# calavera/patrol

Hardware: AMD Instinct MI355X
Metric: bucket-state merges/sec + achieved HBM GB/s at 1/2/4/8 MI355X (higher is better)
Workload: dtype f64; 1 GPU; C2 merge: 100000000 replica messages -> 10000000-bucket table (2^25 slots), Zipf(1.1); keys_per_gpu=10000000, slots_per_gpu=33554432, parallelism=shard1, name_bytes=2-8 (b<id>), world_size=1, full=False, exchange=False, batches_in_hbm=28

## Files before the change

### patrol_amd/csrc/phip_engine.hip

```cpp
#include <sys/random.h>

#include <chrono>
#include <cstdlib>
#include <cstring>
#include <hip/hip_runtime.h>
#include <rocprim/rocprim.hpp>

#include <algorithm>
#include <cstdarg>
#include <cstdio>
#include <cstring>
#include <mutex>
#include <string>
#include <vector>

#include "patrolhip.h"
#include "phip_kernels.hpp"
#include "phip_host.hpp"

using namespace phip;

namespace {

#ifndef PHIP_SORT_BITS
// ... 29 lines not shown
struct DevBuf {
  void* p = nullptr;
  size_t cap = 0;
};

struct Timing {
  const char* name;
  hipEvent_t a, b;
};

}

struct phip_handle {
  int device = 0;
  int ncu = 256;
  u32 ndef = 0;
  bool iso_always = false;
  u32 iso_left = 0;
  bool coll_iso = false;
  bool classify_first = false;
  u32 opt_left = 0;
  struct LastStats {
    uint64_t hot_entries = 0, hot_hits = 0, misses = 0;
    uint64_t ordered = 0;
    uint64_t log_count = 0, log_over = 0;
  } stats;
  hipStream_t stream = nullptr;
  hipStream_t own_stream = nullptr;
  hipStream_t stream2 = nullptr;
  hipStream_t stream3 = nullptr;
  hipStream_t stream4 = nullptr;
  hipEvent_t ev_t4a = nullptr, ev_t4b = nullptr;
  hipEvent_t ev_fork = nullptr, ev_join = nullptr;
  hipEvent_t ev_fork3 = nullptr, ev_join3 = nullptr;
  hipEvent_t ev_gather = nullptr, ev_gather3 = nullptr;
  hipEvent_t ev_pack = nullptr;
  std::mutex mu;
  std::string err;
  u32 L = 0;
  u32 L_open = 0;
  u64 cap = 0;
  u64 max_load = 0;
  u32 load_pct = 90;
  bool grow = true;
  bool small = true;
  u64 grows = 0;
  u64 layout_gen = 1;
  u64 long_need = 0;
  Rec* recs = nullptr;
  u32* aux = nullptr;
  u8* arena = nullptr;
  u64 arena_cap = 0;
  u64 arena_open = 0;
  u64* arena_cursor = nullptr;
  u32* ctr = nullptr;
  u32* ctr_host = nullptr;
  u32* ctr_map = nullptr;
  u32 fpar = 0;
  u64 nfast = 0;
  u64 n_buckets = 0;
  u64 tag_mask = ~0ull;
  u64 seed = 0;
  DevBuf buf[B_COUNT_];
  bool timing = false;
  bool timing_accumulate = false;
  std::vector<Timing> timings;
// ... 336 lines not shown
    cur = nxt;
    nxt = (nxt == retry) ? spare : retry;
  }
  *n_claimed = total;
  if (h->long_need) {
    if ((rc = read_ctr(h)) || (rc = check_flags(h))) return rc;
  }
  return PHIP_OK;
}

int clear_new(phip_handle* h, u32 n_claimed) {
  if (!n_claimed) return PHIP_OK;
  u32* cslot = (u32*)h->buf[B_CSLOT].p;
  Launch l(h, "k_clear_new");
  k_clear_new<<<grid_for(n_claimed), kBlock, 0, h->stream>>>(cslot, n_claimed, table(h));
  HIPCHK(h, hipGetLastError());
  return PHIP_OK;
}

int after_error(phip_handle* h, int rc) {
  if (rc == PHIP_OK) return rc;
  if (h->stream2) (void)hipStreamSynchronize(h->stream2);
  if (h->stream3) (void)hipStreamSynchronize(h->stream3);
  if (h->stream4) (void)hipStreamSynchronize(h->stream4);
  if (rc == PHIP_ERR_HIP) return rc;
  std::string keep = h->err;
  k_clear_new_all<<<grid_for(h->cap), kBlock, 0, h->stream>>>(table(h), h->cap);
  if (hipGetLastError() == hipSuccess) (void)hipStreamSynchronize(h->stream);
  h->err = keep;
  return rc;
}

template <class Src>
int build_hot(phip_handle* h, Src src, u32 n, hipStream_t st, const HotHdr** hdr_out,
              const HotEntry** dir_out) {
  *hdr_out = nullptr;
  *dir_out = nullptr;
  if (n < kHotMinBatch) return PHIP_OK;
  constexpr size_t kCnt = size_t(1) << kHotCntBits;
  const size_t zero_bytes = 2 * kCnt * sizeof(u32) + kHotHist * sizeof(u32) + sizeof(HotHdr);
  u8* base;
  int rc;
  if ((rc = ensure(h, B_HOT, zero_bytes + kHotMax * sizeof(HotEntry), &base))) return rc;
  u32* ckeys = (u32*)base;
  u32* ccnt = ckeys + kCnt;
  u32* hist = ccnt + kCnt;
  HotHdr* hdr = (HotHdr*)(hist + kHotHist);
  HotEntry* dir = (HotEntry*)(hdr + 1);
  HIPCHK(h, hipMemsetAsync(base, 0, zero_bytes, st));
  const u32 stride = std::max<u32>(64, (n + kHotSampleMax - 1) / kHotSampleMax);
  const u32 nsample = (n + stride - 1) / stride;
  {
    Launch l(h, "k_hot_sample", st);
    k_hot_sample<Src><<<grid_for(nsample, kHotSamplePerBlock), 256, 0, st>>>(
        src, n, stride, nsample, table(h), ckeys, ccnt);
  }
  {
    Launch l(h, "k_hot_select", st);
    k_hot_hist<<<grid_for(kCnt), kBlock, 0, st>>>(ccnt, hist);
    k_hot_select<<<1, 256, 0, st>>>(hist, hdr, kHotMax);
    k_hot_build<<<grid_for(kCnt), kBlock, 0, st>>>(ckeys, ccnt, hdr, table(h), dir);
  }
  HIPCHK(h, hipGetLastError());
  *hdr_out = hdr;
  *dir_out = dir;
  return PHIP_OK;
}

inline unsigned fast_grid_on(u32 ncu, u32 n) {
  const u64 tiles = ((u64)n + kFastBlock - 1) / kFastBlock;
  return (unsigned)std::max<u64>(1, std::min<u64>(tiles, (u64)ncu * kFastPerCU));
}
inline unsigned fast_grid(phip_handle* h, u32 n) { return fast_grid_on((u32)h->ncu, n); }

int join_hot(phip_handle* h, const HotHdr* hot);

int sharded(phip_handle* h, BufId base_id, u32 units, u32 per_unit, Sharded* out,
            bool zero = true) {
  int rc;
  out->cap = shard_cap(units, per_unit);
  if ((rc = ensure(h, base_id, (size_t)kShards * out->cap, &out->base)) ||
      (rc = ensure(h, B_MSCNT, 2 * kShards, &out->cnt)))
    return rc;
  if (zero) HIPCHK(h, hipMemsetAsync(out->cnt, 0, kShards * sizeof(u32), h->stream));
  return PHIP_OK;
}

int pack_sharded(phip_handle* h, const Sharded& sh, u32 total_slot, u32* out, u32* total) {
  k_shard_scan<<<1, kShards, 0, h->stream>>>(sh.cnt, h->ctr, total_slot, nullptr, 0, nullptr,
                                             nullptr);
  HIPCHK(h, hipGetLastError());
  int rc;
  if ((rc = read_ctr(h))) return rc;
  *total = h->ctr_host[total_slot];
  if (*total) {
    Launch l(h, "k_shard_compact");
    dim3 grid(grid_for(h->ctr_host[kCtrShardMax]), kShards);
    k_shard_compact<<<grid, 256, 0, h->stream>>>(sh.base, sh.cap, sh.cnt, out);
    HIPCHK(h, hipGetLastError());
  }
  return PHIP_OK;
}

template <class Src>
int fork_hot(phip_handle* h, Src src, u32 n, const HotHdr** hot, const HotEntry** hot_dir);

struct FastFront {
  const HotHdr* hot = nullptr;
  const HotEntry* dir = nullptr;
  u32 par = 0;
  bool iso = false;
  u32* c = nullptr;
  u8* mark = nullptr;
  bool opt = false;
  UndoLog log{};
};

inline bool opt_allowed(const phip_handle* h) {
  return !h->classify_first && h->opt_left == 0 && !h->iso_always && h->iso_left == 0;
}

inline size_t undo_counts(const phip_handle* h) { return (size_t)h->ncu * kFastPerCU * (kFastBlock / 64); }

struct UndoLayout {
  u32 grid, waves, cap;
  u64 halves;
};
inline UndoLayout undo_layout(u32 n, u32 ncu) {
  UndoLayout l;
  l.grid = fast_grid_on(ncu, n);
  l.waves = l.grid * (kFastBlock / 64);
  l.cap = undo_wave_cap(n, l.grid);
  l.halves = (u64)l.waves * l.cap * 2;
  return l;
}

inline u32* fctr(phip_handle* h, u32 par) { return h->ctr + kCtrWords * (1 + par); }

inline u32* fast_counts(phip_handle* h, u32 par) {
  return (u32*)h->buf[B_FSCNT].p + par * 2 * kShards;
}

int dirty_set(phip_handle* h, DirtySet* d, u32** dlist) {
  int rc;
  u64* b;
  if ((rc = ensure(h, B_DTAB, DirtySet::kWords, &b)) || (rc = ensure(h, B_DLIST, kDirtyCap, dlist)))
    return rc;
  *d = DirtySet::at(b);
  return PHIP_OK;
// ... 18 lines not shown
  int rc;
  u32* c;
  out->cap = shard_cap((n + 63) / 64, 64);
  if ((rc = ensure(h, B_MSHARD, (size_t)kShards * out->cap, &out->base)) ||
      (rc = ensure(h, B_FSCNT, 4 * kShards, &c)))
    return rc;
  out->cnt = fast_counts(h, par);
  return PHIP_OK;
}

template <class In, class HotSrc>
int fast_front(phip_handle* h, In in, HotSrc hsrc, u32 n, u8* status, FastFront* ff,
               bool reset = true, int iso = -1, bool opt = false) {
  int rc;
  *ff = FastFront{};
  ff->iso = iso >= 0 ? iso != 0 : (h->iso_always || h->iso_left > 0);
  u32 *c, *dlist = nullptr;
  DirtySet dset;
  if ((rc = ensure(h, B_FSCNT, 4 * kShards, &c))) return rc;
  ff->par = h->fpar ^= 1u;
  ff->c = fctr(h, ff->par);
  ++h->nfast;
  if (reset) {
    k_batch_reset<<<1, kShards, 0, h->stream>>>(ff->c, fast_counts(h, ff->par));
    HIPCHK(h, hipGetLastError());
  }
  if constexpr (In::kSoa) {
    if (opt && iso < 0 && opt_allowed(h)) {
      u32* lc;
      const size_t nw = undo_counts(h);
      if ((rc = ensure(h, B_ULCNT, nw, &lc))) return rc;
      ff->opt = true;
      ff->log.cnt = lc;
      if (n >= kHotMinBatch) HIPCHK(h, hipEventRecord(h->ev_fork, h->stream));
      if (kOptStatus) ff->mark = status;
      else if (status) HIPCHK(h, hipMemsetAsync(status, PHIP_ST_MERGED, n, h->stream));
      if (n >= kHotMinBatch && (rc = fork_hot(h, hsrc, n, &ff->hot, &ff->dir))) return rc;
      return PHIP_OK;
    }
  }
  if ((rc = dirty_set(h, &dset, &dlist))) return rc;
  if (ff->iso) {
    ff->mark = status;
    if (!status) {
      if ((rc = ensure(h, B_DMARK, n, &ff->mark))) return rc;
      HIPCHK(h, hipMemsetAsync(ff->mark, 0, n, h->stream));
    }
  }
  const bool with_hot = n >= kHotMinBatch;
  const bool hot_first = n < (1u << 23);
  if (with_hot) HIPCHK(h, hipEventRecord(h->ev_fork, h->stream));
  if (with_hot && hot_first && (rc = fork_hot(h, hsrc, n, &ff->hot, &ff->dir))) return rc;
  {
    bool done = false;
    if constexpr (In::kSoa) {
      if ((((uintptr_t)in.ma | (uintptr_t)in.mt) & 15) == 0) {
        Launch l(h, "k_classify");
        NamesOffs chk{};
        if constexpr (In::kOffs) chk = in.src;
        k_classify_soa2<<<grid_for((n + 1) / 2), kBlock, 0, h->stream>>>(in.ma, in.mt, in.me, n,
                                                                          ff->c, status, chk,
                                                                          dlist);
        done = true;
      }
    }
    if (!done) {
      if (status) HIPCHK(h, hipMemsetAsync(status, PHIP_ST_MERGED, n, h->stream));
      Launch l(h, "k_classify");
      k_classify<In><<<grid_for(n), kBlock, 0, h->stream>>>(in, n, ff->c, dlist);
    }
  }
  HIPCHK(h, hipGetLastError());
  if (with_hot && !hot_first && (rc = fork_hot(h, hsrc, n, &ff->hot, &ff->dir))) return rc;
  return PHIP_OK;
}

template <class In>
int fast_back(phip_handle* h, In in, u32 n, FastFront& ff, bool queued) {
  u32* miss;
  int rc;
  Sharded msh;
  DirtySet dset{};
  SubBatch sb{};
  u32* dlist = nullptr;
  if ((rc = ensure(h, B_MISS, n, &miss)) || (rc = fast_shards(h, n, ff.par, &msh))) return rc;
  if (ff.iso) {
    if ((rc = dirty_set(h, &dset, &dlist)) || (rc = sub_batch(h, &sb))) return rc;
    Launch l(h, "k_dirty_build");
    k_dirty_build<In><<<1, 1024, 0, h->stream>>>(in, n, ff.c, dlist, dset, table(h));
    HIPCHK(h, hipGetLastError());
  }
  if ((rc = join_hot(h, ff.hot))) return rc;
  if (ff.opt) {
    if constexpr (In::kSoa) {
      const UndoLayout ul = undo_layout(n, (u32)h->ncu);
      ff.log.cap = ul.cap;
      if ((rc = ensure(h, B_ULOG, (size_t)ul.halves, &ff.log.base))) return rc;
      Launch l(h, "k_receive_fast");
      k_receive_fast<In, true><<<ul.grid, kFastBlock, 0, h->stream>>>(
          in, 0, n, table(h), msh, ff.c, ff.hot, ff.dir, nullptr, ff.mark, ff.log);
    }
  } else {
    Launch l(h, "k_receive_fast");
    k_receive_fast<In><<<fast_grid(h, n), kFastBlock, 0, h->stream>>>(
        in, 0, n, table(h), msh, ff.c, ff.hot, ff.dir, ff.iso ? dset.key : nullptr, ff.mark,
        UndoLog{});
  }
  HIPCHK(h, hipGetLastError());
  if (ff.iso) {
    {
      Launch l(h, "k_dirty_pass");
      const unsigned g = (unsigned)std::max<u64>(
          1, std::min<u64>(((u64)n + 1023) / 1024, (u64)h->ncu * 2));
      k_dirty_pass<In><<<g, 1024, 0, h->stream>>>(in, n, ff.c, ff.mark, dset.key, table(h), msh);
      HIPCHK(h, hipGetLastError());
    }
    k_batch_end<In><<<1, kShards, 0, h->stream>>>(
        in, ff.c, dset.key, table(h),
        SubOut{sb.off, sb.len, sb.a, sb.t, sb.e, sb.map, kSubBatchCap}, msh.cnt, h->ctr_map,
        kCtrWords, queued ? fast_counts(h, ff.par ^ 1u) : nullptr, fctr(h, ff.par ^ 1u));
  } else {
    k_shard_scan<<<1, kShards, 0, h->stream>>>(msh.cnt, ff.c, kCtrMiss, h->ctr_map, kCtrWords,
                                               queued ? fast_counts(h, ff.par ^ 1u) : nullptr,
                                               fctr(h, ff.par ^ 1u));
  }
  HIPCHK(h, hipGetLastError());
  HIPCHK(h, hipEventRecord(h->ev_ctr, h->stream));
  if (!queued) HIPCHK(h, hipEventSynchronize(h->ev_ctr));
  return PHIP_OK;
}

constexpr u32 kIsoKeep = 256;
constexpr u32 kOptBackoff = 256;

bool opt_failed(phip_handle* h, u32 n) {
  h->stats.log_count = h->ctr_host[kCtrLogCount];
  h->stats.log_over = h->ctr_host[kCtrLogOver];
  if (h->stats.log_over) h->opt_left = kOptBackoff;
  return h->ctr_host[kCtrDirty] < n || h->ctr_host[kCtrStop] < n || h->stats.log_over != 0;
}

// ... 20 lines not shown
    HIPCHK(h, hipGetLastError());
  }
  const u32 nd = h->ctr_host[kCtrNDirty];
  const bool iso = iso_ran && nd != 0 && nd <= kDirtyCap;
  *first_dirty = iso ? n : std::min<u32>(h->ctr_host[kCtrDirty], n);
  if (h->ctr_host[kCtrDirty] < n) h->iso_left = kIsoKeep;
  else if (h->iso_left) --h->iso_left;
  h->coll_iso = iso_ran;
  h->ndef = iso ? h->ctr_host[kCtrNDefer] : 0;
  h->stats.ordered = 0;
  h->stats.hot_entries = h->ctr_host[kCtrHotEntries];
  h->stats.hot_hits = h->ctr_host[kCtrHotHits];
  h->stats.misses = *nmiss;
  return PHIP_OK;
}

template <class In, class HotSrc>
int fast_apply(phip_handle* h, In in, HotSrc hsrc, u32 n, u8* status, u32* first_dirty,
               u32* nmiss, int iso = -1, bool opt = false) {
  int rc;
  FastFront ff;
  if ((rc = fast_front(h, in, hsrc, n, status, &ff, true, iso, opt)) ||
      (rc = fast_back(h, in, n, ff, false)))
    return rc;
  if (ff.opt && opt_failed(h, n)) {
    if ((rc = undo_pass(h, n, ff.log)) || (rc = fast_front(h, in, hsrc, n, status, &ff, true, iso)) ||
        (rc = fast_back(h, in, n, ff, false)))
      return rc;
  }
  return fast_collect(h, n, ff.par, first_dirty, nmiss, ff.iso, ff.opt);
}

template <class Src>
int fork_hot(phip_handle* h, Src src, u32 n, const HotHdr** hot, const HotEntry** hot_dir);

template <class Src>
int dedupe_names(phip_handle* h, Src src, const u32* list, u32 n, u32** out, u32* nout) {
  int rc;
  u32 setbits = 1;
  while ((1ull << setbits) < 2ull * n) ++setbits;
  u64* set;
  Sharded dsh;
  if ((rc = ensure(h, B_DSET, size_t(1) << setbits, &set)) ||
      (rc = ensure(h, B_DEDUP, n, out)) ||
      (rc = sharded(h, B_MSHARD, grid_for(n), kBlock, &dsh)))
    return rc;
  HIPCHK(h, hipMemsetAsync(set, 0, (size_t(1) << setbits) * sizeof(u64), h->stream));
  {
    Launch l(h, "k_dedupe");
    k_dedupe<Src><<<grid_for(n), kBlock, 0, h->stream>>>(src, n, list, table(h), set, setbits, dsh);
    HIPCHK(h, hipGetLastError());
  }
  return pack_sharded(h, dsh, kCtrAux, *out, nout);
}

template <class Src>
int finish_many_misses(phip_handle* h, Src src, const uint64_t* a, const uint64_t* t,
                       const int64_t* e, u32 nmiss, u32 prefix, i64 now, u8* status, u32* nmiss2) {
  u32* miss = (u32*)h->buf[B_MISS].p;
  int rc;
  u32 *dedup, nd = 0;
  if ((rc = dedupe_names(h, src, miss, nmiss, &dedup, &nd))) return rc;
  u32 n_claimed = 0;
  if ((rc = insert_names(h, src, dedup, nd, nullptr, now, &n_claimed, nullptr, true))) return rc;
  if (status) {
    Launch l(h, "k_first_seen");
    k_first_seen<Src><<<grid_for(nmiss), kBlock, 0, h->stream>>>(src, nmiss, miss, table(h));
    HIPCHK(h, hipGetLastError());
  }
// ... 14 lines not shown
int finish_misses(phip_handle* h, Src src, const uint64_t* a, const uint64_t* t, const int64_t* e,
                  u32 nmiss, u32 prefix, i64 now, u8* status) {
  if (nmiss == 0) return PHIP_OK;
  int rc;
  if (nmiss >= kManyMisses &&
      (rc = finish_many_misses(h, src, a, t, e, nmiss, prefix, now, status, &nmiss)))
    return rc;
  if (nmiss == 0) return PHIP_OK;
  u32* miss = (u32*)h->buf[B_MISS].p;
  u32 n_claimed = 0;
  if ((rc = insert_names(h, src, miss, nmiss, nullptr, now, &n_claimed))) return rc;
  HIPCHK(h, hipMemsetAsync(h->ctr + kCtrMiss, 0, sizeof(u32), h->stream));
  u32* miss2;
  if ((rc = ensure(h, B_MISS2, nmiss, &miss2))) return rc;
  {
    Launch l(h, "k_receive_list");
    k_receive_list<Src><<<grid_for(nmiss), kBlock, 0, h->stream>>>(
        src, a, t, e, nmiss, miss, table(h), status, miss2, h->ctr);
  }
  HIPCHK(h, hipGetLastError());
  {
    Launch l(h, "k_mark_created");
    k_mark_created<Src><<<grid_for(nmiss), kBlock, 0, h->stream>>>(src, nmiss, miss, table(h),
                                                                    status);
  }
  HIPCHK(h, hipGetLastError());
  if ((rc = read_ctr(h))) return rc;
  if (const u32 left = h->ctr_host[kCtrMiss])
    return set_err(h, PHIP_ERR_INVALID, "internal: %u names missing after insert", left);
  return clear_new(h, n_claimed);
}

template <class Src>
int fork_hot(phip_handle* h, Src src, u32 n, const HotHdr** hot, const HotEntry** hot_dir) {
  *hot = nullptr;
  *hot_dir = nullptr;
  if (n < kHotMinBatch) return PHIP_OK;
  HIPCHK(h, hipStreamWaitEvent(h->stream2, h->ev_fork, 0));
  int rc;
  if ((rc = build_hot(h, src, n, h->stream2, hot, hot_dir))) return rc;
  HIPCHK(h, hipEventRecord(h->ev_join, h->stream2));
  return PHIP_OK;
}

int join_hot(phip_handle* h, const HotHdr* hot) {
  if (hot) HIPCHK(h, hipStreamWaitEvent(h->stream, h->ev_join, 0));
  return PHIP_OK;
}


#define PHIP_OUT_DISPATCH(mask, CALL) \
  switch (mask) {                     \
    case 0: CALL(0); break;           \
    case 1: CALL(1); break;           \
    case 2: CALL(2); break;           \
    case 3: CALL(3); break;           \
    case 4: CALL(4); break;           \
    case 5: CALL(5); break;           \
    case 6: CALL(6); break;           \
    case 7: CALL(7); break;           \
    case 8: CALL(8); break;           \
    case 9: CALL(9); break;           \
    case 10: CALL(10); break;         \
    case 11: CALL(11); break;         \
    case 12: CALL(12); break;         \
    case 13: CALL(13); break;         \
    case 14: CALL(14); break;         \
    default: CALL(15); break;         \
  }

template <class Src>
int resolve_all(phip_handle* h, Src src, u32 n, const int64_t* now_arr, i64 now0, u32** slot_out,
                u32* n_claimed, SortVals sv = SortVals{nullptr, 0, nullptr}) {
  u32 *slot, *miss;
  int rc;
  Sharded rsh;
  if ((rc = ensure(h, B_SLOT, n, &slot)) || (rc = ensure(h, B_MISS, n, &miss)) ||
      (rc = sharded(h, B_MSHARD, grid_for(n), kBlock, &rsh)))
    return rc;
// ... 2080 lines not shown
```

### patrol_amd/csrc/phip_kernels.hpp

```cpp
#pragma once
#include <type_traits>

#include "phip_device.hpp"

namespace phip {

constexpr int kBlock = 256;

template <bool NT, class T>
__device__ inline T ld(const T* p) {
  if constexpr (NT) return __builtin_nontemporal_load(p);
  else return *p;
}

__device__ inline u64 load_be64(const u8* p) {
  u64 v = 0;
#pragma unroll
  for (int k = 0; k < 8; ++k) v = (v << 8) | p[k];
  return v;
}

struct NamesOffs {
  const u8* blob;
  const u32* offs;
// ... 444 lines not shown
  u64 b1 = sh ? (w1 >> sh) | (w2 << (64 - sh)) : w1;
  u64 b2 = sh ? (w2 >> sh) | (w3 << (64 - sh)) : w2;
  b1 = low_bytes(b1, len - 8);
  b2 = len > 16 ? low_bytes(b2, len - 16) : 0;
  u32 lo = (u32)kFnvOffset, hi = (u32)(kFnvOffset >> 32);
  fnv_word32(lo, hi, b0, 8);
  fnv_word32(lo, hi, b1, len - 8);
  if (len > 16) fnv_word32(lo, hi, b2, len - 16);
  nm.h = ((u64)hi << 32) | lo; nm.len = len; nm.off = off;
  nm.w0 = (u64)len | (b0 << 16);
  nm.w1 = (b0 >> 48) | (b1 << 16);
  nm.w2 = (b1 >> 48) | (b2 << 16);
}

__device__ inline u64 enc_replica_nz(u64 b) {
  const u64 mag = b & ~kSign;
  const u64 e = (b >> 63) ? kInfBits - mag : kInfBits + mag + (mag != 0);
  return mag > kInfBits ? 0ull : e;
}

#ifndef PHIP_HOT_MAX
#define PHIP_HOT_MAX 736
#endif
#ifndef PHIP_HOT_LDS
#define PHIP_HOT_LDS 4096
#endif
constexpr u32 kHotMax = PHIP_HOT_MAX;
constexpr u32 kHotLds = PHIP_HOT_LDS;
constexpr u32 kRouteHotMax = 512;
static_assert(kHotLds * 2 >= kRouteHotMax * 3 && kHotLds * 2 >= kHotMax * 3, "LDS lookup load");
constexpr u32 kHotCntBits = 18;
constexpr u32 kHotSampleMax = 1u << 17;
constexpr u32 kHotSamplePerBlock = 1024;
constexpr u32 kHotHist = 4096;
constexpr u32 kHotMinCount = 8;
constexpr u32 kHotMinBatch = 1u << 16;
constexpr u32 kRouteMinBatch = 1u << 20;
#ifndef PHIP_MANY_MISSES
#define PHIP_MANY_MISSES (1u << 16)
#endif
constexpr u32 kManyMisses = PHIP_MANY_MISSES;

constexpr u32 kHotTailName = 40;
constexpr u32 kHotTailWords = (kHotTailName - 16) / 8;
struct HotEntry {
  u64 tag, w0, w1, w2;
  u64 tail[kHotTailWords];
  u32 slot, aoff;
};
struct HotHdr {
  u32 n;
  u32 thresh;
  u32 pad[14];
};

__device__ inline u32 hot_home(u64 tag) { return (u32)(tag ^ (tag >> 29)) & (kHotLds - 1); }

template <class Src>
__global__ __launch_bounds__(256) void k_hot_sample(Src src, u32 n, u32 stride, u32 nsample, Table T,
                                                    u32* __restrict__ ckeys, u32* __restrict__ ccnt) {
  constexpr u32 kPer = kHotSamplePerBlock / 256;
  constexpr u32 kL = 2 * kHotSamplePerBlock;
  __shared__ u32 lkey[kL], lcnt[kL];
  for (u32 e = threadIdx.x; e < kL; e += 256) { lkey[e] = 0; lcnt[e] = 0; }
  __syncthreads();
  for (u32 r = 0; r < kPer; ++r) {
    const u32 j = blockIdx.x * kHotSamplePerBlock + r * 256 + threadIdx.x;
    const u64 i = (u64)j * stride;
    if (j >= nsample || i >= n) continue;
    u64 off; u32 len;
    src.template get<true>((u32)i, off, len);
    Name nm;
    load_name_wide<true>(src.blob, off, len, nm);
    u32 s;
    Rec rec;
    if (probe(T, nm, src.blob, &s, &rec) != kFound) continue;
    u32 h = (s * 2654435761u) & (kL - 1);
    for (;;) {
      const u32 old = atomicCAS(&lkey[h], 0u, s + 1);
      if (old == 0 || old == s + 1) { atomicAdd(&lcnt[h], 1u); break; }
      h = (h + 1) & (kL - 1);
    }
  }
  __syncthreads();
  constexpr u32 mask = (1u << kHotCntBits) - 1;
  for (u32 e = threadIdx.x; e < kL; e += 256) {
    const u32 key = lkey[e];
    if (!key) continue;
    u32 h = ((key - 1) * 2654435761u) >> (32 - kHotCntBits);
    for (u32 k = 0; k <= mask; ++k) {
      const u32 old = atomicCAS(&ckeys[h], 0u, key);
      if (old == 0 || old == key) { atomicAdd(&ccnt[h], lcnt[e]); break; }
      h = (h + 1) & mask;
    }
  }
}

__global__ void k_hot_hist(const u32* __restrict__ ccnt, u32* __restrict__ hist) {
  const u32 e = blockIdx.x * blockDim.x + threadIdx.x;
  if (e >= (1u << kHotCntBits)) return;
  const u32 c = ccnt[e];
  if (c >= kHotMinCount) atomicAdd(&hist[c < kHotHist ? c : kHotHist - 1], 1u);
}

__global__ __launch_bounds__(256) void k_hot_select(const u32* __restrict__ hist, HotHdr* hdr,
                                                    u32 maxn) {
  constexpr u32 kPer = kHotHist / 256;
  __shared__ u32 part[256];
  __shared__ u32 best;
  const u32 t = threadIdx.x;
  u32 s = 0;
  for (u32 k = 0; k < kPer; ++k) s += hist[t * kPer + k];
  part[t] = s;
  if (t == 0) best = kHotHist;
  __syncthreads();
  u32 run = 0;
  for (u32 u = t + 1; u < 256; ++u) run += part[u];
  u32 lo = kHotHist;
  for (int b = (int)kPer - 1; b >= 0; --b) {
    run += hist[t * kPer + b];
    if (run <= maxn) lo = t * kPer + b;
  }
  atomicMin(&best, lo);
  __syncthreads();
  if (t == 0) {
    hdr->n = 0;
    hdr->thresh = best > kHotMinCount ? best : kHotMinCount;
  }
}

__global__ void k_hot_build(const u32* __restrict__ ckeys, const u32* __restrict__ ccnt, HotHdr* hdr,
                            Table T, HotEntry* __restrict__ dir) {
  const u32 e = blockIdx.x * blockDim.x + threadIdx.x;
  if (e >= (1u << kHotCntBits)) return;
  const u32 c = ccnt[e];
  if (c < kHotMinCount || c < hdr->thresh) return;
  const u32 idx = atomicAdd(&hdr->n, 1u);
  if (idx >= kHotMax) return;
  const u32 s = ckeys[e] - 1;
  const Rec r = load_rec(&T.recs[s]);
  HotEntry d;
  const bool arena = (r.name0 & 0xFFu) > kInlineName;
  d.tag = r.tag;
  d.w0 = arena ? (r.name0 & 0xFFu) : (r.name0 & ~0xFF00ull);
  d.w1 = r.name1;
  d.w2 = r.name2;
  d.slot = s;
  d.aoff = arena ? (u32)(r.name0 >> 32) : 0u;
  const u32 len = (u32)(r.name0 & 0xFFu);
  for (u32 k = 0; k < kHotTailWords; ++k) d.tail[k] = 0;
  if (arena && len <= kHotTailName) {
    const u64 a0 = (r.name0 >> 32) + 16;
    const u64* p = reinterpret_cast<const u64*>(T.arena + (a0 & ~7ull));
    const u32 sh = (u32)(a0 & 7) * 8, lastw = ((u32)(a0 & 7) + len - 17) >> 3;
    for (u32 k = 0; 8 * k < len - 16; ++k) {
      const u32 m = len - 16 - 8 * k;
      d.tail[k] = low_bytes(str_word(p, sh, k, lastw), m);
    }
  }
  dir[idx] = d;
}

#ifndef PHIP_FAST_BLOCK
#define PHIP_FAST_BLOCK 1024
#endif
#ifndef PHIP_FAST_PER_CU
#define PHIP_FAST_PER_CU 2
#endif
constexpr u32 kFastBlock = PHIP_FAST_BLOCK;
constexpr u32 kFastPerCU = PHIP_FAST_PER_CU;

template <class Src>
struct SoaIn {
  Src src;
  const uint64_t* ma;
  const uint64_t* mt;
  const int64_t* me;
  static constexpr bool kSoa = true;
  __device__ inline const u8* blob() const { return src.blob; }
  struct PreOffs { u32 a, b; };
  struct PreGen { u64 off; u32 len; };
  static constexpr bool kOffs = std::is_same<Src, NamesOffs>::value;
  using Pre = typename std::conditional<kOffs, PreOffs, PreGen>::type;
  __device__ inline Pre pre(u32 i) const {
    Pre p;
    if constexpr (kOffs) {
      p.a = ld<true>(src.offs + i);
      p.b = ld<true>(src.offs + i + 1);
    } else {
      src.template get<true>(i, p.off, p.len);
    }
    return p;
  }
// ... 284 lines not shown
  u64x2* base = nullptr;
  u32* cnt = nullptr;
  u32 cap = 0;
};
__host__ __device__ inline u32 fast_wave_chunks(u32 n, u32 grid) {
  const u32 nchunks = (n + 63) / 64, kw = kFastBlock / 64;
  if (grid % 8 == 0) {
    const u32 per = (nchunks + 7) / 8, waves = grid / 8 * kw;
    return (per + waves - 1) / waves;
  }
  return (nchunks + grid * kw - 1) / (grid * kw);
}
constexpr u32 kUndoSlack = 24;
__host__ __device__ inline u32 undo_wave_cap(u32 n, u32 grid) {
  return fast_wave_chunks(n, grid) * 32 + kUndoSlack + kUndoFlushReserve;
}
__device__ inline u32 lane_rank(u64 m) {
  return __builtin_amdgcn_mbcnt_hi((u32)(m >> 32), __builtin_amdgcn_mbcnt_lo((u32)m, 0u));
}
__device__ inline void undo_store(u64x2* p, u32 slot, u64 a, u64 t, i64 e) {
#if PHIP_UNDO_NT
  __builtin_nontemporal_store(u64x2{(u64)slot, a}, p);
  __builtin_nontemporal_store(u64x2{t, (u64)e}, p + 1);
#else
  p[0] = u64x2{(u64)slot, a};
  p[1] = u64x2{t, (u64)e};
#endif
}

template <class In, bool Opt = false>
__global__ __launch_bounds__(kFastBlock) __attribute__((amdgpu_waves_per_eu(8, 8))) void k_receive_fast(
    In in, u32 lo, u32 n, Table T, Sharded miss, u32* ctr,
    const HotHdr* __restrict__ hot, const HotEntry* __restrict__ hot_dir, const u64* dtab,
    u8* __restrict__ mark, UndoLog ulog) {
  __shared__ u32 hslot[kHotLds];
  __shared__ u64 htag[kHotMax], hw0[kHotMax], hw1[kHotMax], hw2[kHotMax];
  __shared__ u32 hrec[kHotMax], haoff[kHotMax];
  __shared__ u64 htail[kHotTailWords][kHotMax];
  __shared__ u64 hmax[3][kHotMax];
  __shared__ u32 hhits;
  __shared__ u32 hlog[2];

  const u32 ndr = !Opt && dtab ? ctr[kCtrNDirty] : 0u;
  const bool iso = !Opt && ndr != 0 && ndr <= kDirtyCap;
  if constexpr (!Opt) n = min(n, iso ? ctr[kCtrStop] : min(ctr[kCtrStop], ctr[kCtrDirty]));
  if (n <= lo) return;
  const u32 nh = hot ? min(hot->n, kHotMax) : 0u;
  for (u32 j = threadIdx.x; j < kHotLds; j += kFastBlock) hslot[j] = 0;
  for (u32 j = threadIdx.x; j < kHotMax; j += kFastBlock) {
    hmax[0][j] = 0; hmax[1][j] = 0; hmax[2][j] = 0;
  }
  if (threadIdx.x == 0) hhits = 0;
  if (Opt && threadIdx.x < 2) hlog[threadIdx.x] = 0;
  __syncthreads();
  for (u32 j = threadIdx.x; j < nh; j += kFastBlock) {
    const HotEntry d = hot_dir[j];
    htag[j] = d.tag; hw0[j] = d.w0; hw1[j] = d.w1; hw2[j] = d.w2;
    hrec[j] = d.slot | (iso && (rec_flags(T.recs[d.slot]) & kRecDirty) ? 0x80000000u : 0u);
    haoff[j] = d.aoff;
    for (u32 k = 0; k < kHotTailWords; ++k) htail[k][j] = d.tail[k];
    u32 hs = hot_home(d.tag);
    while (atomicCAS(&hslot[hs], 0u, j + 1) != 0) hs = (hs + 1) & (kHotLds - 1);
  }
  __syncthreads();

  constexpr u32 kWaves = kFastBlock / 64;
  const u32 lane = threadIdx.x & 63;
  u32 nchunks = (n + 63) / 64;
  u32 hits = 0;
  const u32 wave = __builtin_amdgcn_readfirstlane(threadIdx.x / 64);
  u32 cstride, chunk;
  if (gridDim.x % 8 == 0) {
    const u32 per = (nchunks - lo / 64 + 7) / 8;
    const u32 c0 = lo / 64 + (blockIdx.x % 8) * per;
    nchunks = min(nchunks, c0 + per);
// ... 3431 lines not shown
```

Measured before the change: 50.35 billion merges/s.

## Fuse hot-key sampling, selection and directory build into one last-block kernel

Replaces the four-kernel hot-key pipeline (sample, hist, select, build) with a single k_hot_dir kernel. The last finishing workgroup, detected with an atomic counter, computes the histogram, threshold and directory from a compact candidate list. In the opt path, the status memset is folded into extra blocks of that kernel, which runs on the main stream instead of being forked. Re-zeroing of the count tables moves into k_receive_fast so the next batch can skip the separate memset. This cuts launch count and memset traffic, at the cost of relying on a fragile inter-block completion protocol and adding stores to the hot merge kernel.

```diff
diff --git a/patrol_amd/csrc/phip_engine.hip b/patrol_amd/csrc/phip_engine.hip
--- a/patrol_amd/csrc/phip_engine.hip
+++ b/patrol_amd/csrc/phip_engine.hip
@@ -85,6 +85,7 @@
   hipStream_t stream4 = nullptr;
   hipEvent_t ev_t4a = nullptr, ev_t4b = nullptr;
   hipEvent_t ev_fork = nullptr, ev_join = nullptr;
+  void* hot_clean = nullptr;
   hipEvent_t ev_fork3 = nullptr, ev_join3 = nullptr;
   hipEvent_t ev_gather = nullptr, ev_gather3 = nullptr;
   hipEvent_t ev_pack = nullptr;
@@ -487,38 +488,47 @@
 }
 
 template <class Src>
-int build_hot(phip_handle* h, Src src, u32 n, hipStream_t st, const HotHdr** hdr_out,
-              const HotEntry** dir_out) {
+int build_hot(phip_handle* h, Src src, u32 n, hipStream_t st, u8* status, const HotHdr** hdr_out,
+              const HotEntry** dir_out, void** zero_out) {
   *hdr_out = nullptr;
   *dir_out = nullptr;
+  *zero_out = nullptr;
   if (n < kHotMinBatch) return PHIP_OK;
   constexpr size_t kCnt = size_t(1) << kHotCntBits;
-  const size_t zero_bytes = 2 * kCnt * sizeof(u32) + kHotHist * sizeof(u32) + sizeof(HotHdr);
   u8* base;
   int rc;
-  if ((rc = ensure(h, B_HOT, zero_bytes + kHotMax * sizeof(HotEntry), &base))) return rc;
+  if ((rc = ensure(h, B_HOT, kHotZeroBytes + kHotCandMax * sizeof(u32) + sizeof(HotHdr) +
+                                 kHotMax * sizeof(HotEntry), &base)))
+    return rc;
   u32* ckeys = (u32*)base;
   u32* ccnt = ckeys + kCnt;
-  u32* hist = ccnt + kCnt;
-  HotHdr* hdr = (HotHdr*)(hist + kHotHist);
+  u32* sync = ccnt + kCnt;
+  u32* cand = sync + kHotSyncWords;
+  HotHdr* hdr = (HotHdr*)(cand + kHotCandMax);
   HotEntry* dir = (HotEntry*)(hdr + 1);
-  HIPCHK(h, hipMemsetAsync(base, 0, zero_bytes, st));
+  if (h->hot_clean != base) HIPCHK(h, hipMemsetAsync(base, 0, kHotZeroBytes, st));
+  h->hot_clean = nullptr;
   const u32 stride = std::max<u32>(64, (n + kHotSampleMax - 1) / kHotSampleMax);
   const u32 nsample = (n + stride - 1) / stride;
   {
-    Launch l(h, "k_hot_sample", st);
-    k_hot_sample<Src><<<grid_for(nsample, kHotSamplePerBlock), 256, 0, st>>>(
-        src, n, stride, nsample, table(h), ckeys, ccnt);
-  }
-  {
-    Launch l(h, "k_hot_select", st);
-    k_hot_hist<<<grid_for(kCnt), kBlock, 0, st>>>(ccnt, hist);
-    k_hot_select<<<1, 256, 0, st>>>(hist, hdr, kHotMax);
-    k_hot_build<<<grid_for(kCnt), kBlock, 0, st>>>(ckeys, ccnt, hdr, table(h), dir);
+    Launch l(h, "k_hot_dir", st);
+    if (status) {
+      constexpr unsigned kT = kHotAloneThreads;
+      const unsigned nblk = grid_for(nsample, kT);
+      const unsigned fill =
+          std::min<unsigned>(grid_for(n, kT * 64), 1024 / kT * (unsigned)h->ncu);
+      k_hot_dir<Src, kT, 1><<<nblk + fill, kT, 0, st>>>(
+          src, n, stride, nsample, table(h), ckeys, ccnt, sync, cand, hdr, dir, nblk, status);
+    } else {
+      const unsigned nblk = grid_for(nsample, kHotSamplePerBlock);
+      k_hot_dir<Src, 256, 4><<<nblk, 256, 0, st>>>(
+          src, n, stride, nsample, table(h), ckeys, ccnt, sync, cand, hdr, dir, nblk, nullptr);
+    }
   }
   HIPCHK(h, hipGetLastError());
   *hdr_out = hdr;
   *dir_out = dir;
+  *zero_out = base;
   return PHIP_OK;
 }
 
@@ -528,7 +538,6 @@
 }
 inline unsigned fast_grid(phip_handle* h, u32 n) { return fast_grid_on((u32)h->ncu, n); }
 
-int join_hot(phip_handle* h, const HotHdr* hot);
 
 int sharded(phip_handle* h, BufId base_id, u32 units, u32 per_unit, Sharded* out,
             bool zero = true) {
@@ -557,12 +566,11 @@
   return PHIP_OK;
 }
 
-template <class Src>
-int fork_hot(phip_handle* h, Src src, u32 n, const HotHdr** hot, const HotEntry** hot_dir);
-
 struct FastFront {
   const HotHdr* hot = nullptr;
   const HotEntry* dir = nullptr;
+  void* hot_zero = nullptr;
+  bool hot_join = false;
   u32 par = 0;
   bool iso = false;
   u32* c = nullptr;
@@ -570,6 +578,9 @@
   bool opt = false;
   UndoLog log{};
 };
+template <class Src>
+int fork_hot(phip_handle* h, Src src, u32 n, FastFront* ff);
+int join_hot(phip_handle* h, const FastFront& ff);
 
 inline bool opt_allowed(const phip_handle* h) {
   return !h->classify_first && h->opt_left == 0 && !h->iso_always && h->iso_left == 0;
@@ -654,10 +665,15 @@
       if ((rc = ensure(h, B_ULCNT, nw, &lc))) return rc;
       ff->opt = true;
       ff->log.cnt = lc;
-      if (n >= kHotMinBatch) HIPCHK(h, hipEventRecord(h->ev_fork, h->stream));
       if (kOptStatus) ff->mark = status;
-      else if (status) HIPCHK(h, hipMemsetAsync(status, PHIP_ST_MERGED, n, h->stream));
-      if (n >= kHotMinBatch && (rc = fork_hot(h, hsrc, n, &ff->hot, &ff->dir))) return rc;
+      u8* fill = kOptStatus ? nullptr : status;
+      if (n >= kHotMinBatch && fill)
+        return build_hot(h, hsrc, n, h->stream, fill, &ff->hot, &ff->dir, &ff->hot_zero);
+      if (fill) HIPCHK(h, hipMemsetAsync(fill, PHIP_ST_MERGED, n, h->stream));
+      if (n >= kHotMinBatch) {
+        HIPCHK(h, hipEventRecord(h->ev_fork, h->stream));
+        return fork_hot(h, hsrc, n, ff);
+      }
       return PHIP_OK;
     }
   }
@@ -672,7 +688,7 @@
   const bool with_hot = n >= kHotMinBatch;
   const bool hot_first = n < (1u << 23);
   if (with_hot) HIPCHK(h, hipEventRecord(h->ev_fork, h->stream));
-  if (with_hot && hot_first && (rc = fork_hot(h, hsrc, n, &ff->hot, &ff->dir))) return rc;
+  if (with_hot && hot_first && (rc = fork_hot(h, hsrc, n, ff))) return rc;
   {
     bool done = false;
     if constexpr (In::kSoa) {
@@ -693,7 +709,7 @@
     }
   }
   HIPCHK(h, hipGetLastError());
-  if (with_hot && !hot_first && (rc = fork_hot(h, hsrc, n, &ff->hot, &ff->dir))) return rc;
+  if (with_hot && !hot_first && (rc = fork_hot(h, hsrc, n, ff))) return rc;
   return PHIP_OK;
 }
 
@@ -712,7 +728,7 @@
     k_dirty_build<In><<<1, 1024, 0, h->stream>>>(in, n, ff.c, dlist, dset, table(h));
     HIPCHK(h, hipGetLastError());
   }
-  if ((rc = join_hot(h, ff.hot))) return rc;
+  if ((rc = join_hot(h, ff))) return rc;
   if (ff.opt) {
     if constexpr (In::kSoa) {
       const UndoLayout ul = undo_layout(n, (u32)h->ncu);
@@ -720,15 +736,17 @@
       if ((rc = ensure(h, B_ULOG, (size_t)ul.halves, &ff.log.base))) return rc;
       Launch l(h, "k_receive_fast");
       k_receive_fast<In, true><<<ul.grid, kFastBlock, 0, h->stream>>>(
-          in, 0, n, table(h), msh, ff.c, ff.hot, ff.dir, nullptr, ff.mark, ff.log);
+          in, 0, n, table(h), msh, ff.c, ff.hot, ff.dir, nullptr, ff.mark, ff.log,
+          (uint4*)ff.hot_zero);
     }
   } else {
     Launch l(h, "k_receive_fast");
     k_receive_fast<In><<<fast_grid(h, n), kFastBlock, 0, h->stream>>>(
         in, 0, n, table(h), msh, ff.c, ff.hot, ff.dir, ff.iso ? dset.key : nullptr, ff.mark,
-        UndoLog{});
+        UndoLog{}, (uint4*)ff.hot_zero);
   }
   HIPCHK(h, hipGetLastError());
+  if (ff.hot_zero) h->hot_clean = ff.hot_zero;
   if (ff.iso) {
     {
       Launch l(h, "k_dirty_pass");
@@ -815,9 +833,6 @@
 }
 
 template <class Src>
-int fork_hot(phip_handle* h, Src src, u32 n, const HotHdr** hot, const HotEntry** hot_dir);
-
-template <class Src>
 int dedupe_names(phip_handle* h, Src src, const u32* list, u32 n, u32** out, u32* nout) {
   int rc;
   u32 setbits = 1;
@@ -898,19 +913,18 @@
 }
 
 template <class Src>
-int fork_hot(phip_handle* h, Src src, u32 n, const HotHdr** hot, const HotEntry** hot_dir) {
-  *hot = nullptr;
-  *hot_dir = nullptr;
+int fork_hot(phip_handle* h, Src src, u32 n, FastFront* ff) {
   if (n < kHotMinBatch) return PHIP_OK;
   HIPCHK(h, hipStreamWaitEvent(h->stream2, h->ev_fork, 0));
   int rc;
-  if ((rc = build_hot(h, src, n, h->stream2, hot, hot_dir))) return rc;
+  if ((rc = build_hot(h, src, n, h->stream2, nullptr, &ff->hot, &ff->dir, &ff->hot_zero))) return rc;
   HIPCHK(h, hipEventRecord(h->ev_join, h->stream2));
-  return PHIP_OK;
-}
-
-int join_hot(phip_handle* h, const HotHdr* hot) {
-  if (hot) HIPCHK(h, hipStreamWaitEvent(h->stream, h->ev_join, 0));
+  ff->hot_join = true;
+  return PHIP_OK;
+}
+
+int join_hot(phip_handle* h, const FastFront& ff) {
+  if (ff.hot_join) HIPCHK(h, hipStreamWaitEvent(h->stream, h->ev_join, 0));
   return PHIP_OK;
 }
 
diff --git a/patrol_amd/csrc/phip_kernels.hpp b/patrol_amd/csrc/phip_kernels.hpp
--- a/patrol_amd/csrc/phip_kernels.hpp
+++ b/patrol_amd/csrc/phip_kernels.hpp
@@ -500,8 +500,15 @@
 constexpr u32 kHotCntBits = 18;
 constexpr u32 kHotSampleMax = 1u << 17;
 constexpr u32 kHotSamplePerBlock = 1024;
+#ifndef PHIP_HOT_ALONE
+#define PHIP_HOT_ALONE 256
+#endif
+constexpr u32 kHotAloneThreads = PHIP_HOT_ALONE;
 constexpr u32 kHotHist = 4096;
 constexpr u32 kHotMinCount = 8;
+constexpr u32 kHotCandMax = kHotSampleMax / kHotMinCount;
+constexpr u32 kHotSyncWords = 16;
+constexpr size_t kHotZeroBytes = (2 * (size_t(1) << kHotCntBits) + kHotSyncWords) * sizeof(u32);
 constexpr u32 kHotMinBatch = 1u << 16;
 constexpr u32 kRouteMinBatch = 1u << 20;
 #ifndef PHIP_MANY_MISSES
@@ -524,88 +531,7 @@
 
 __device__ inline u32 hot_home(u64 tag) { return (u32)(tag ^ (tag >> 29)) & (kHotLds - 1); }
 
-template <class Src>
-__global__ __launch_bounds__(256) void k_hot_sample(Src src, u32 n, u32 stride, u32 nsample, Table T,
-                                                    u32* __restrict__ ckeys, u32* __restrict__ ccnt) {
-  constexpr u32 kPer = kHotSamplePerBlock / 256;
-  constexpr u32 kL = 2 * kHotSamplePerBlock;
-  __shared__ u32 lkey[kL], lcnt[kL];
-  for (u32 e = threadIdx.x; e < kL; e += 256) { lkey[e] = 0; lcnt[e] = 0; }
-  __syncthreads();
-  for (u32 r = 0; r < kPer; ++r) {
-    const u32 j = blockIdx.x * kHotSamplePerBlock + r * 256 + threadIdx.x;
-    const u64 i = (u64)j * stride;
-    if (j >= nsample || i >= n) continue;
-    u64 off; u32 len;
-    src.template get<true>((u32)i, off, len);
-    Name nm;
-    load_name_wide<true>(src.blob, off, len, nm);
-    u32 s;
-    Rec rec;
-    if (probe(T, nm, src.blob, &s, &rec) != kFound) continue;
-    u32 h = (s * 2654435761u) & (kL - 1);
-    for (;;) {
-      const u32 old = atomicCAS(&lkey[h], 0u, s + 1);
-      if (old == 0 || old == s + 1) { atomicAdd(&lcnt[h], 1u); break; }
-      h = (h + 1) & (kL - 1);
-    }
-  }
-  __syncthreads();
-  constexpr u32 mask = (1u << kHotCntBits) - 1;
-  for (u32 e = threadIdx.x; e < kL; e += 256) {
-    const u32 key = lkey[e];
-    if (!key) continue;
-    u32 h = ((key - 1) * 2654435761u) >> (32 - kHotCntBits);
-    for (u32 k = 0; k <= mask; ++k) {
-      const u32 old = atomicCAS(&ckeys[h], 0u, key);
-      if (old == 0 || old == key) { atomicAdd(&ccnt[h], lcnt[e]); break; }
-      h = (h + 1) & mask;
-    }
-  }
-}
-
-__global__ void k_hot_hist(const u32* __restrict__ ccnt, u32* __restrict__ hist) {
-  const u32 e = blockIdx.x * blockDim.x + threadIdx.x;
-  if (e >= (1u << kHotCntBits)) return;
-  const u32 c = ccnt[e];
-  if (c >= kHotMinCount) atomicAdd(&hist[c < kHotHist ? c : kHotHist - 1], 1u);
-}
-
-__global__ __launch_bounds__(256) void k_hot_select(const u32* __restrict__ hist, HotHdr* hdr,
-                                                    u32 maxn) {
-  constexpr u32 kPer = kHotHist / 256;
-  __shared__ u32 part[256];
-  __shared__ u32 best;
-  const u32 t = threadIdx.x;
-  u32 s = 0;
-  for (u32 k = 0; k < kPer; ++k) s += hist[t * kPer + k];
-  part[t] = s;
-  if (t == 0) best = kHotHist;
-  __syncthreads();
-  u32 run = 0;
-  for (u32 u = t + 1; u < 256; ++u) run += part[u];
-  u32 lo = kHotHist;
-  for (int b = (int)kPer - 1; b >= 0; --b) {
-    run += hist[t * kPer + b];
-    if (run <= maxn) lo = t * kPer + b;
-  }
-  atomicMin(&best, lo);
-  __syncthreads();
-  if (t == 0) {
-    hdr->n = 0;
-    hdr->thresh = best > kHotMinCount ? best : kHotMinCount;
-  }
-}
-
-__global__ void k_hot_build(const u32* __restrict__ ckeys, const u32* __restrict__ ccnt, HotHdr* hdr,
-                            Table T, HotEntry* __restrict__ dir) {
-  const u32 e = blockIdx.x * blockDim.x + threadIdx.x;
-  if (e >= (1u << kHotCntBits)) return;
-  const u32 c = ccnt[e];
-  if (c < kHotMinCount || c < hdr->thresh) return;
-  const u32 idx = atomicAdd(&hdr->n, 1u);
-  if (idx >= kHotMax) return;
-  const u32 s = ckeys[e] - 1;
+__device__ inline HotEntry hot_entry(const Table& T, u32 s) {
   const Rec r = load_rec(&T.recs[s]);
   HotEntry d;
   const bool arena = (r.name0 & 0xFFu) > kInlineName;
@@ -626,7 +552,238 @@
       d.tail[k] = low_bytes(str_word(p, sh, k, lastw), m);
     }
   }
-  dir[idx] = d;
+  return d;
+}
+
+__device__ inline u32 ld_co32(const u32* p) {
+  return __hip_atomic_load(p, __ATOMIC_RELAXED, __HIP_MEMORY_SCOPE_AGENT);
+}
+__device__ inline void st_co32(u32* p, u32 v) {
+  __hip_atomic_store(p, v, __ATOMIC_RELAXED, __HIP_MEMORY_SCOPE_AGENT);
+}
+
+template <class Src, u32 kThreads, u32 kRounds>
+__global__ __launch_bounds__(kThreads) void k_hot_dir(Src src, u32 n, u32 stride, u32 nsample,
+                                                      Table T, u32* ckeys, u32* ccnt, u32* sync,
+                                                      u32* cand, HotHdr* hdr,
+                                                      HotEntry* __restrict__ dir, u32 nblk,
+                                                      u8* __restrict__ status) {
+  constexpr u32 kPerBlock = kThreads * kRounds;
+  constexpr u32 kL = 2 * kPerBlock;
+  static_assert(kHotHist % kThreads == 0 && 4096 % kThreads == 0, "the last workgroup's shares");
+  constexpr u32 kWords = 2 * kL > kHotHist ? 2 * kL : kHotHist;
+  __shared__ u32 lds[kWords];
+  __shared__ u32 part[kThreads];
+  __shared__ u32 sel[kHotMax];
+  __shared__ u32 best, nsel, last;
+  if (blockIdx.x >= nblk) {
+    constexpr u32 b4 = PHIP_ST_MERGED * 0x01010101u;
+    const u64 head = min((u64)n, (u64)(-(uintptr_t)status & 15));
+    const u64 n16 = (n - head) / 16;
+    uint4* body = reinterpret_cast<uint4*>(status + head);
+    const u64 step = (u64)(gridDim.x - nblk) * kThreads;
+    for (u64 k = (u64)(blockIdx.x - nblk) * kThreads + threadIdx.x; k < n16; k += step)
+      body[k] = uint4{b4, b4, b4, b4};
+    if (blockIdx.x == nblk) {
+      if (threadIdx.x < head) status[threadIdx.x] = PHIP_ST_MERGED;
+      const u64 done = head + n16 * 16;
+      if (done + threadIdx.x < n) status[done + threadIdx.x] = PHIP_ST_MERGED;
+    }
+    return;
+  }
+  u32* lkey = lds;
+  u32* lcnt = lds + kL;
+  for (u32 e = threadIdx.x; e < 2 * kL; e += kThreads) lds[e] = 0;
+  __syncthreads();
+  for (u32 r = 0; r < kRounds; ++r) {
+    const u32 j = blockIdx.x * kPerBlock + r * kThreads + threadIdx.x;
+    const u64 i = (u64)j * stride;
+    if (j >= nsample || i >= n) continue;
+    u64 off; u32 len;
+    src.template get<true>((u32)i, off, len);
+    Name nm;
+    load_name_wide<true>(src.blob, off, len, nm);
+    u32 s;
+    Rec rec;
+    if (probe(T, nm, src.blob, &s, &rec) != kFound) continue;
+    u32 h = (s * 2654435761u) & (kL - 1);
+    for (;;) {
+      const u32 old = atomicCAS(&lkey[h], 0u, s + 1);
+      if (old == 0 || old == s + 1) { atomicAdd(&lcnt[h], 1u); break; }
+      h = (h + 1) & (kL - 1);
+    }
+  }
+  __syncthreads();
+  constexpr u32 mask = (1u << kHotCntBits) - 1;
+  constexpr u32 kE = kL / kThreads;
+  u32 key[kE], cnt[kE], hh[kE], before[kE];
+#pragma unroll
+  for (u32 k = 0; k < kE; ++k) {
+    key[k] = lkey[k * kThreads + threadIdx.x];
+    cnt[k] = lcnt[k * kThreads + threadIdx.x];
+    hh[k] = ((key[k] - 1) * 2654435761u) >> (32 - kHotCntBits);
+    before[k] = ~0u;
+  }
+  for (u32 tries = 0; tries <= mask; ++tries) {
+    u32 old[kE];
+#pragma unroll
+    for (u32 k = 0; k < kE; ++k)
+      if (key[k] && before[k] == ~0u) old[k] = atomicCAS(&ckeys[hh[k]], 0u, key[k]);
+    bool again = false;
+#pragma unroll
+    for (u32 k = 0; k < kE; ++k) {
+      if (!key[k] || before[k] != ~0u) continue;
+      if (old[k] == 0 || old[k] == key[k]) before[k] = atomicAdd(&ccnt[hh[k]], cnt[k]);
+      else { hh[k] = (hh[k] + 1) & mask; again = true; }
+    }
+    if (!again) break;
+  }
+  u32 ncross = 0;
+#pragma unroll
+  for (u32 k = 0; k < kE; ++k) {
+    const bool cross = key[k] && before[k] < kHotMinCount && before[k] + cnt[k] >= kHotMinCount;
+    if (!cross) key[k] = 0;
+    ncross += cross;
+  }
+  if (ncross) {
+    u32 at = atomicAdd(&sync[1], ncross);
+#pragma unroll
+    for (u32 k = 0; k < kE; ++k)
+      if (key[k] && at < kHotCandMax) st_co32(&cand[at++], hh[k]);
+  }
+  asm volatile("s_waitcnt vmcnt(0)" ::: "memory");
+  __syncthreads();
+  if (threadIdx.x == 0) {
+    const u32 t = __hip_atomic_fetch_add(&sync[0], 1u, __ATOMIC_RELAXED, __HIP_MEMORY_SCOPE_AGENT);
+    last = t == nblk - 1;
+    if (last) {
+      __builtin_amdgcn_fence(__ATOMIC_ACQUIRE, "agent");
+      asm volatile("s_waitcnt vmcnt(0)" ::: "memory");
+    }
+  }
+  __syncthreads();
+  if (!last) return;
+
+  constexpr u32 kU = 4096 / kThreads;
+  static_assert(4096 <= kHotCandMax, "the list entries read before its length");
+  u32 hh0[kU];
+#pragma unroll
+  for (u32 k = 0; k < kU; ++k) hh0[k] = ld_co32(&cand[k * kThreads + threadIdx.x]);
+  const u32 ncand = min(ld_co32(&sync[1]), kHotCandMax);
+#pragma unroll
+  for (u32 k = 0; k < kU; ++k) hh0[k] = k * kThreads + threadIdx.x < ncand ? hh0[k] & mask : ~0u;
+  u32* hist = lds;
+  for (u32 e = threadIdx.x; e < kHotHist; e += kThreads) hist[e] = 0;
+  if (threadIdx.x == 0) { best = kHotHist; nsel = 0; }
+  __syncthreads();
+  auto counts = [&](const u32 (&hh)[kU], u32 (&cc)[kU], u32 (&kk)[kU]) {
+#pragma unroll
+    for (u32 k = 0; k < kU; ++k) {
+      cc[k] = hh[k] != ~0u ? ld_co32(&ccnt[hh[k]]) : 0u;
+      kk[k] = hh[k] != ~0u ? ld_co32(&ckeys[hh[k]]) : 0u;
+    }
+  };
+  auto load = [&](u32 base, u32 (&cc)[kU], u32 (&kk)[kU]) {
+    u32 hh[kU];
+#pragma unroll
+    for (u32 k = 0; k < kU; ++k) {
+      const u32 c = base + k * kThreads + threadIdx.x;
+      hh[k] = c < ncand ? ld_co32(&cand[c]) & mask : ~0u;
+    }
+    counts(hh, cc, kk);
+  };
+  auto count = [&](const u32 (&cc)[kU]) {
+#pragma unroll
+    for (u32 k = 0; k < kU; ++k)
+      if (cc[k] >= kHotMinCount) atomicAdd(&hist[cc[k] < kHotHist ? cc[k] : kHotHist - 1], 1u);
+  };
+  u32 cc0[kU], kk0[kU];
+  counts(hh0, cc0, kk0);
+  count(cc0);
+  for (u32 base = kThreads * kU; base < ncand; base += kThreads * kU) {
+    u32 cc[kU], kk[kU];
+    load(base, cc, kk);
+    count(cc);
+  }
+  __syncthreads();
+  {
+    constexpr u32 kBins = kHotHist / kThreads;
+    const u32 t = threadIdx.x;
+    u32 s = 0;
+    for (u32 k = 0; k < kBins; ++k) s += hist[t * kBins + k];
+    part[t] = s;
+    __syncthreads();
+    u32 run = 0;
+    for (u32 u = t + 1; u < kThreads; ++u) run += part[u];
+    u32 lo = kHotHist;
+    for (int b = (int)kBins - 1; b >= 0; --b) {
+      run += hist[t * kBins + b];
+      if (run <= kHotMax) lo = t * kBins + b;
+    }
+    atomicMin(&best, lo);
+    __syncthreads();
+  }
+  const u32 thresh = best > kHotMinCount ? best : kHotMinCount;
+  auto pick = [&](const u32 (&cc)[kU], const u32 (&kk)[kU]) {
+#pragma unroll
+    for (u32 k = 0; k < kU; ++k) {
+      if (cc[k] < thresh) continue;
+      const u32 idx = atomicAdd(&nsel, 1u);
+      if (idx < kHotMax) sel[idx] = kk[k] - 1;
+    }
+  };
+  pick(cc0, kk0);
+  for (u32 base = kThreads * kU; base < ncand; base += kThreads * kU) {
+    u32 cc[kU], kk[kU];
+    load(base, cc, kk);
+    pick(cc, kk);
+  }
+  __syncthreads();
+  const u32 ns = min(nsel, kHotMax);
+#pragma unroll
+  for (u32 k = 0; k < (kHotMax + kThreads - 1) / kThreads; ++k) {
+    const u32 j = k * kThreads + threadIdx.x;
+    if (j < ns) dir[j] = hot_entry(T, sel[j]);
+  }
+  if (threadIdx.x == 0) {
+    hdr->n = nsel;
+    hdr->thresh = thresh;
+    st_co32(&sync[0], 0u);
+    st_co32(&sync[1], 0u);
+  }
+}
+
+__global__ void k_hot_hist(const u32* __restrict__ ccnt, u32* __restrict__ hist) {
+  const u32 e = blockIdx.x * blockDim.x + threadIdx.x;
+  if (e >= (1u << kHotCntBits)) return;
+  const u32 c = ccnt[e];
+  if (c >= kHotMinCount) atomicAdd(&hist[c < kHotHist ? c : kHotHist - 1], 1u);
+}
+
+__global__ __launch_bounds__(256) void k_hot_select(const u32* __restrict__ hist, HotHdr* hdr,
+                                                    u32 maxn) {
+  constexpr u32 kPer = kHotHist / 256;
+  __shared__ u32 part[256];
+  __shared__ u32 best;
+  const u32 t = threadIdx.x;
+  u32 s = 0;
+  for (u32 k = 0; k < kPer; ++k) s += hist[t * kPer + k];
+  part[t] = s;
+  if (t == 0) best = kHotHist;
+  __syncthreads();
+  u32 run = 0;
+  for (u32 u = t + 1; u < 256; ++u) run += part[u];
+  u32 lo = kHotHist;
+  for (int b = (int)kPer - 1; b >= 0; --b) {
+    run += hist[t * kPer + b];
+    if (run <= maxn) lo = t * kPer + b;
+  }
+  atomicMin(&best, lo);
+  __syncthreads();
+  if (t == 0) {
+    hdr->n = 0;
+    hdr->thresh = best > kHotMinCount ? best : kHotMinCount;
+  }
 }
 
 #ifndef PHIP_FAST_BLOCK
@@ -977,7 +1134,7 @@
 __global__ __launch_bounds__(kFastBlock) __attribute__((amdgpu_waves_per_eu(8, 8))) void k_receive_fast(
     In in, u32 lo, u32 n, Table T, Sharded miss, u32* ctr,
     const HotHdr* __restrict__ hot, const HotEntry* __restrict__ hot_dir, const u64* dtab,
-    u8* __restrict__ mark, UndoLog ulog) {
+    u8* __restrict__ mark, UndoLog ulog, uint4* __restrict__ hot_zero) {
   __shared__ u32 hslot[kHotLds];
   __shared__ u64 htag[kHotMax], hw0[kHotMax], hw1[kHotMax], hw2[kHotMax];
   __shared__ u32 hrec[kHotMax], haoff[kHotMax];
@@ -986,6 +1143,10 @@
   __shared__ u32 hhits;
   __shared__ u32 hlog[2];
 
+  if (hot_zero)
+    for (u32 k = blockIdx.x * kFastBlock + threadIdx.x; k < kHotZeroBytes / sizeof(uint4);
+         k += gridDim.x * kFastBlock)
+      hot_zero[k] = uint4{0, 0, 0, 0};
   const u32 ndr = !Opt && dtab ? ctr[kCtrNDirty] : 0u;
   const bool iso = !Opt && ndr != 0 && ndr <= kDirtyCap;
   if constexpr (!Opt) n = min(n, iso ? ctr[kCtrStop] : min(ctr[kCtrStop], ctr[kCtrDirty]));
```

Result: faster. 52.33 billion merges/s (median of 6 runs) (+3.9%).
